# seung-lab/crackle

Hardware: AMD Instinct MI355X
Metric: voxels/s encode+decode, 1024x1024x512 uint32; bit-exact .ckl bytes (higher is better)
Workload: dtype u32

## Files before the change

### crackle_amd/_lib.py

```python
import ctypes as C
import os

HERE = os.path.dirname(os.path.abspath(__file__))
LIB_PATH = os.path.join(HERE, "libcrackle_amd_tuning.so" if os.environ.get("CKL_TUNING_LIB") else
                        ("libcrackle_amd_%s.so" % os.environ["CKL_LIB_AB"]) if os.environ.get("CKL_LIB_AB") else "libcrackle_amd.so")

CKL_OK, CKL_ERR_FORMAT, CKL_ERR_RUNTIME, CKL_ERR_ARG, CKL_ERR_NO_DEVICE, CKL_ERR_CRC = range(6)
MEM_HOST, MEM_DEVICE = 0, 1
CKL_DUST_BINARY_IMAGE, CKL_DUST_INVERT = 1, 2
CKL_ERODE_KEEP_BORDER = 1


class HeaderInfo(C.Structure):
  _fields_ = [
    ("format_version", C.c_uint32), ("label_format", C.c_uint32), ("crack_format", C.c_uint32),
    ("is_signed", C.c_uint32), ("data_width", C.c_uint32), ("stored_data_width", C.c_uint32),
    ("sx", C.c_uint32), ("sy", C.c_uint32), ("sz", C.c_uint32),
    ("fortran_order", C.c_uint32), ("markov_model_order", C.c_uint32), ("is_sorted", C.c_uint32),
    ("num_label_bytes", C.c_uint64), ("header_bytes", C.c_uint64),
  ]


MERGE_UNIQUE_FN = C.CFUNCTYPE(C.c_int, C.c_void_p, C.POINTER(C.c_uint64), C.c_uint64, C.POINTER(C.c_void_p), C.POINTER(C.c_uint64))

# ... 51 lines not shown
    C.c_int, C.c_int, C.c_uint64, C.c_int, C.c_int, C.c_int64,
    C.POINTER(EncodeOverrides), C.POINTER(C.c_void_p), C.POINTER(C.c_uint64)]),
  "ckl_encoder_stats": (C.c_int, [
    C.c_void_p, C.c_void_p, C.c_int64, C.c_int64, C.c_int64,
    C.POINTER(C.c_uint64), C.POINTER(C.c_uint64), C.POINTER(C.c_uint64), C.POINTER(C.c_uint64)]),
  "ckl_encoder_markov_stats": (C.c_int, [
    C.c_void_p, C.c_void_p, C.c_int64, C.c_int64, C.c_int64, C.c_int, C.c_uint64, C.c_void_p]),
  "ckl_encoder_components": (C.c_int, [
    C.c_void_p, C.c_void_p, C.c_int64, C.c_int64, C.c_int64, C.c_uint32, C.c_void_p, C.c_void_p]),
  "ckl_encoder_components_device": (C.c_int, [
    C.c_void_p, C.c_void_p, C.c_int64, C.c_int64, C.c_int64, C.c_uint32, C.c_void_p, C.c_void_p]),
  "ckl_encoder_pin_labels": (C.c_int, [
    C.c_void_p, C.c_void_p, C.c_void_p, C.c_int64, C.c_int64, C.c_int64, C.c_void_p,
    C.c_int, C.c_int, C.c_int64, C.POINTER(C.c_void_p), C.POINTER(C.c_uint64)]),
  "ckl_pins_rows_first": (C.c_int, [C.c_void_p, C.c_void_p, C.c_void_p, C.c_int64, C.c_int64, C.c_int64, C.c_int64, C.c_uint64, C.c_void_p, C.c_void_p, C.c_void_p]),
  "ckl_pins_rows_best": (C.c_int, [C.c_void_p, C.c_void_p, C.c_void_p, C.c_int64, C.c_int64, C.c_int64, C.c_int64, C.c_uint64, C.c_void_p, C.c_void_p]),
  "ckl_pins_rows_extent": (C.c_int, [C.c_void_p, C.c_void_p, C.c_void_p, C.c_int64, C.c_int64, C.c_int64, C.c_int64, C.c_uint64, C.c_void_p, C.c_void_p, C.c_void_p, C.c_void_p]),
  "ckl_pins_rows_ids": (C.c_int, [C.c_void_p, C.c_void_p, C.c_int64, C.c_int64, C.c_int64, C.c_int64, C.c_uint64, C.c_void_p, C.c_void_p, C.c_void_p, C.c_void_p]),
  "ckl_pins_rows_section": (C.c_int, [C.c_void_p, C.c_int64, C.c_int64, C.c_int64, C.c_uint64, C.c_void_p, C.c_void_p, C.c_void_p, C.c_void_p, C.c_void_p, C.c_void_p, C.c_void_p,
                                       C.c_int, C.c_int, C.c_int64, C.POINTER(C.c_void_p), C.POINTER(C.c_uint64)]),
  "ckl_encoder_walk_step_kinds": (C.c_int, [C.c_void_p, C.POINTER(C.c_uint32), C.c_uint32, C.POINTER(C.c_uint32)]),
  "ckl_encoder_last_timing": (C.c_int, [C.c_void_p, C.POINTER(C.c_float), C.POINTER(C.c_float)]),
  "ckl_encoder_walk_paths": (C.c_int, [C.c_void_p, C.POINTER(C.c_uint32), C.POINTER(C.c_uint32)]),
  "ckl_encoder_destroy": (None, [C.c_void_p]),
  "ckl_pin_labels_host": (C.c_int, [
    C.c_void_p, C.c_int, C.c_void_p, C.c_int64, C.c_int64, C.c_int64, C.c_void_p,
    C.c_int, C.c_int, C.c_int64, C.POINTER(C.c_void_p), C.POINTER(C.c_uint64)]),
  "ckl_zstack": (C.c_int, [C.POINTER(C.c_char_p), C.POINTER(C.c_uint64), C.c_uint64, C.POINTER(C.c_void_p), C.POINTER(C.c_uint64)]),
  "ckl_decoder_check": (C.c_int, [C.c_void_p, C.c_void_p, C.c_uint64]),
  "ckl_decoder_vcg": (C.c_int, [C.c_void_p, C.c_void_p, C.c_uint64, C.c_int]),
  "ckl_voxel_connectivity_graph": (C.c_int, [C.c_void_p, C.c_uint64, C.c_int, C.c_int, C.c_void_p, C.c_uint64]),
  "ckl_voxel_connectivity_graph_range": (C.c_int, [C.c_void_p, C.c_uint64, C.c_int64, C.c_int64, C.c_int, C.c_int, C.c_void_p, C.c_uint64]),
  "ckl_point_cloud": (C.c_int, [
    C.c_void_p, C.c_uint64, C.c_int64, C.c_int64, C.c_void_p, C.c_uint64, C.c_int, C.c_int, C.c_int,
    C.POINTER(C.c_void_p), C.POINTER(C.c_void_p), C.POINTER(C.c_void_p), C.POINTER(C.c_uint64)]),
  "ckl_reencode_markov": (C.c_int, [C.c_void_p, C.c_uint64, C.c_int, C.c_int, C.POINTER(C.c_void_p), C.POINTER(C.c_uint64)]),
  "ckl_recompress": (C.c_int, [C.c_void_p, C.c_uint64, C.c_int, C.c_int, C.POINTER(C.c_void_p), C.POINTER(C.c_uint64)]),
  "ckl_erode": (C.c_int, [C.c_void_p, C.c_uint64, C.c_int, C.c_int, C.c_int, C.c_int, C.POINTER(C.c_void_p), C.POINTER(C.c_uint64)]),
  "ckl_dilate": (C.c_int, [C.c_void_p, C.c_uint64, C.c_int, C.c_int, C.c_int, C.c_int, C.POINTER(C.c_void_p), C.POINTER(C.c_uint64)]),
  "ckl_decoder_crack_planes": (C.c_int, [C.c_void_p, C.POINTER(C.c_void_p), C.POINTER(C.c_void_p), C.POINTER(C.c_uint32), C.POINTER(C.c_uint64)]),
  "ckl_zsplit": (C.c_int, [C.c_void_p, C.c_uint64, C.c_int64, C.c_int64, C.POINTER(C.c_void_p), C.POINTER(C.c_uint64)]),
  "ckl_encoder_defer_codes": (C.c_int, [C.c_void_p, C.c_int]),
  "ckl_encoder_codes_to_host": (C.c_int, [C.c_void_p, C.c_void_p, C.c_uint64, C.POINTER(C.c_uint64)]),
  "ckl_host_register": (C.c_int, [C.c_void_p, C.c_uint64]),
  "ckl_host_unregister": (C.c_int, [C.c_void_p]),
  "ckl_array_equal": (C.c_int, [C.c_void_p, C.c_uint64, C.c_void_p, C.c_uint64, C.c_int, C.POINTER(C.c_int)]),
# ... 72 lines not shown
```

### crackle_amd/csrc/ckl_encode.hip

```cpp
#include "ckl_encoder.hpp"
#include "ckl_decoder.hpp"
#include "ckl_runs.hpp"
#include "ckl_strips.hpp"
#include "ckl_trail.hpp"
#include "ckl_recompress.hpp"

#include <algorithm>
#include <atomic>
#include <chrono>
#include <functional>
#include <memory>
#include <mutex>

namespace ckl {

using namespace dev;

template <typename LABEL>
__global__ void __launch_bounds__(kBlock) k_stats(const LABEL* __restrict__ labels, uint64_t voxels, unsigned long long* __restrict__ out ) {
	__shared__ unsigned long long s_max[kWaves], s_pairs[kWaves];
	unsigned long long mx = 0, pairs = 0;
	const uint64_t stride = static_cast<uint64_t>(gridDim.x) * kBlock;
	for (uint64_t i = static_cast<uint64_t>(blockIdx.x) * kBlock + threadIdx.x; i < voxels; i += stride) {
		const LABEL v = labels[i];
		if (static_cast<unsigned long long>(v) > mx) mx = v;
		if (i > 0) pairs += (labels[i - 1] == v);
	}
// ... 477 lines not shown
				const uint4 v = *reinterpret_cast<const uint4*>(fcode + g0);
				const uint32_t w4[4] = { v.x, v.y, v.z, v.w };
#pragma unroll
				for (uint32_t j = 0; j < 16; j++) c[j] = static_cast<uint8_t>(w4[j >> 2] >> (8u * (j & 3u)));
			}
			else {
#pragma unroll
				for (uint32_t j = 0; j < 16; j++) c[j] = g0 + j < nvalid ? fcode[g0 + j] : 0;
			}
			uint32_t prev = g0 ? fcode[g0 - 1] : 0u;
			uint32_t enc = 0;
#pragma unroll
			for (uint32_t j = 0; j < 16; j++) {
				if (g0 + j < nvalid) enc |= ((c[j] - prev) & 3u) << (2 * j);
				prev = c[j];
			}
			if (4u * w + 4u <= nbytes) reinterpret_cast<uint32_t*>(out)[w] = enc;
			else for (uint32_t k = 4u * w; k < nbytes; k++) out[k] = static_cast<uint8_t>(enc >> (8u * (k - 4u * w)));
		}
		if (tid == 0) a.payload_len[zi] = nbytes;
	}
}

__device__ __forceinline__ uint32_t markov_ctx(const uint8_t* d, uint32_t g, int order) {
	uint32_t ctx = 0;
	for (int j = 1; j <= order; j++) {
		const uint32_t v = (g >= static_cast<uint32_t>(j)) ? d[g - j] : 0u;
		ctx |= v << (2 * (order - j));
	}
	return ctx;
}

__global__ void __launch_bounds__(kBlock) k_markov_hist(
	const uint8_t* __restrict__ dcode, const uint64_t* __restrict__ cbase, const uint32_t* __restrict__ n_valid,
	int order, uint32_t* __restrict__ hist, uint32_t lds_entries
) {
	extern __shared__ uint32_t s_hist[];
	const uint32_t zi = blockIdx.x;
	const uint8_t* d = dcode + cbase[zi];
	const uint32_t n = n_valid[zi];
	const uint32_t entries = 4u << (2 * order);
	const bool local = entries <= lds_entries;
	if (local) {
		for (uint32_t i = threadIdx.x; i < entries; i += kBlock) s_hist[i] = 0;
		__syncthreads();
	}
// ... 665 lines not shown
	if (st && !po.empty()) *st = v;
	e.graph_permissible = on_device ? static_cast<int64_t>(v.pairs) < static_cast<int64_t>(static_cast<uint64_t>(sx) * sy * sz) / 2 : format == GraphFormat::PERMISSIBLE;
}

enum class CrackGoal { HISTOGRAM, CODES };
struct CrackRequest {
	CrackGoal goal = CrackGoal::CODES;
	bool permissible = false;
	int markov_order = 0;
	const std::vector<uint8_t>* model = nullptr;
	bool reuse_trail = false;
	std::function<void()> overlap;
};
struct CrackResult {
	std::vector<uint32_t> code_len;
	uint64_t total = 0;
	bool any_chain = false;
	std::vector<uint32_t> hist;
	std::vector<uint8_t> model;
};

inline size_t trail_walk_lds(uint32_t max_special) { return (static_cast<size_t>(max_special) + 256) * 16 + 1024; }

FinishArgs finish_args(const ckl_encoder& e, int64_t sx, int64_t sy, int markov_order) {
	FinishArgs fa;
	fa.sx = static_cast<int>(sx); fa.sy = static_cast<int>(sy);
	fa.xw = byte_width(static_cast<uint64_t>(sx) + 1); fa.yw = byte_width(static_cast<uint64_t>(sy) + 1);
	fa.markov = markov_order ? 1u : 0u;
	fa.cbase = e.d_cbase.p; fa.kbase = e.d_kbase.p;
	fa.n_chains = e.d_n_chains.p; fa.n_raw = e.d_n_raw.p; fa.n_valid = e.d_n_valid.p;
	fa.cp = e.d_cp.p; fa.chain_node = e.d_chain_node.p; fa.chain_off = e.d_chain_off.p; fa.chain_clen = e.d_chain_clen.p;
	fa.chain_order = e.d_chain_order.p; fa.chain_dst = e.d_chain_dst.p; fa.chain_vstart = e.d_chain_vstart.p;
	fa.fcode = e.d_fcode.p; fa.dcode = e.d_dcode.p;
	fa.pbase = e.d_pbase.p; fa.payload = e.d_payload.p; fa.bbase = e.d_bbase.p; fa.boc = e.d_boc.p;
	fa.payload_len = e.d_payload_len.p; fa.boc_len = e.d_boc_len.p;
	fa.z0 = 0;
	return fa;
}

TrailArgs trail_args(const ckl_encoder& e, int64_t sx, int64_t sy, uint32_t ns) {
	const uint64_t nverts = static_cast<uint64_t>(sx + 1) * (sy + 1);
	TrailArgs ta;
	ta.adjm = e.d_adjm.p; ta.adjm_stride = e.adjm_stride; ta.mtx2 = e.mtx2; ta.tiles_x = e.tiles_x; ta.tiles_y = e.tiles_y;
	ta.planeV = plane_v(e); ta.planeH = plane_h(e, ns); ta.row_words = e.row_words; ta.plane_words = e.plane_words;
	ta.sx = static_cast<uint32_t>(sx); ta.sy = static_cast<uint32_t>(sy); ta.inv = e.graph_permissible ? 0xFFFFFFFFu : 0u;
	ta.sxe = static_cast<uint32_t>(sx + 1); ta.sye = static_cast<uint32_t>(sy + 1); ta.nverts = static_cast<uint32_t>(nverts);
// ... 48 lines not shown
	const std::vector<uint32_t> errs = download(e.d_slice_err.p, ns, e.stream);
	for (uint32_t zi = 0; zi < ns; zi++) if (errs[zi]) throw Error(CKL_ERR_RUNTIME, "crackle_amd: crack walk scratch overflow on z=" + std::to_string(zi));
}

CrackResult crack_pass(ckl_encoder& e, int64_t sx, int64_t sy, int64_t sz, const CrackRequest& rq) {
	hipStream_t s = e.stream;
	const uint32_t ns = static_cast<uint32_t>(sz);
	const uint64_t nverts = static_cast<uint64_t>(sx + 1) * (sy + 1);
	const int markov_order = rq.markov_order;
	const bool reuse_trail = rq.reuse_trail;
	if (rq.goal == CrackGoal::HISTOGRAM && (!markov_order || rq.model)) throw Error(CKL_ERR_RUNTIME, "crackle_amd: internal: a markov histogram needs an order and no model");
	CrackResult result;
	e.d_slice_err.ensure(ns);
	const bool prezeroed = e.trail_zeroed && !reuse_trail;
	e.trail_zeroed = false;
	if (prezeroed) CKL_HIP(hipStreamWaitEvent(s, e.ev_prezero, 0));
	if (!reuse_trail && !prezeroed) CKL_HIP(hipMemsetAsync(e.d_slice_err.p, 0, ns * sizeof(uint32_t), s));

	std::vector<uint64_t> cbase(ns), sbase(ns), kbase(ns);
	std::vector<uint32_t> ccap(ns), scap(ns), kcap(ns), max_steps(ns);
	std::vector<uint64_t> nbase(ns), cobase(ns), ibase(ns);
	std::vector<uint32_t> ncap(ns), cocap(ns), icap(ns);
	uint64_t ctot = 0, stot = 0, ktot = 0, ntot = 0, cotot = 0, itot = 0;
	uint32_t max_ncap = 0, max_cocap = 0, max_icap = 0, max_special = 0;
	bool any = false;
	for (uint32_t zi = 0; zi < ns; zi++) {
		const uint64_t E = crack_edges(e, sx, sy, zi, rq.permissible);
		any = any || E > 0;
		const uint64_t cc = ((7 * E + 16 + 15) / 16) * 16;
		if (cc > 0xFFFFFFF0ull) throw Error(CKL_ERR_RUNTIME, "crackle_amd: slice has too many crack edges");
		cbase[zi] = ctot; ccap[zi] = static_cast<uint32_t>(cc); ctot += cc;
		max_steps[zi] = static_cast<uint32_t>(E + 1);
		const uint64_t nc = ((static_cast<uint64_t>(e.count_special[zi]) + e.count_corner[zi] + 16) / 16) * 16;
		if (nc >= (1ull << 28)) throw Error(CKL_ERR_RUNTIME, "crackle_amd: slice has too many crack vertices");
		nbase[zi] = ntot; ncap[zi] = static_cast<uint32_t>(nc); ntot += nc;
		cobase[zi] = cotot; cocap[zi] = e.count_corner[zi]; cotot += e.count_corner[zi];
		const uint64_t ic = 7 * nc + 16;
		ibase[zi] = itot; icap[zi] = static_cast<uint32_t>(ic); itot += ic;
		sbase[zi] = stot; scap[zi] = static_cast<uint32_t>(2 * nc + 4); stot += 2 * nc + 4;
		kbase[zi] = ktot; kcap[zi] = static_cast<uint32_t>(nc); ktot += nc;
		max_ncap = std::max<uint32_t>(max_ncap, ncap[zi]);
		max_cocap = std::max<uint32_t>(max_cocap, cocap[zi]);
		max_icap = std::max<uint32_t>(max_icap, icap[zi]);
		max_special = std::max<uint32_t>(max_special, e.count_special[zi]);
	}
	result.any_chain = any;
	if (g_ht && g_ht->on) {
		uint32_t over = 0;
		for (uint32_t zi = 0; zi < ns; zi++) over += e.count_special[zi] > 3584u;
		fprintf(stderr, "[ckl trail nodes] max special %u, slices above 3584: %u of %u\n", max_special, over, ns);
	}
	HT_MARK("c:caps");

	UploadPacker tables;
	tables.add(e.d_cbase, cbase); tables.add(e.d_ccap, ccap);
	tables.add(e.d_sbase, sbase); tables.add(e.d_scap, scap);
	tables.add(e.d_kbase, kbase); tables.add(e.d_kcap, kcap);
	e.d_cp.ensure(ctot); e.d_fcode.ensure(ctot);
	if (markov_order) e.d_dcode.ensure(ctot);
	e.d_stack_node.ensure(stot); e.d_stack_code.ensure(stot);
	e.d_chain_node.ensure(ktot); e.d_chain_off.ensure(ktot); e.d_chain_clen.ensure(ktot);
	e.d_chain_order.ensure(ktot); e.d_chain_dst.ensure(ktot); e.d_chain_vstart.ensure(ktot);
	e.d_n_chains.ensure(ns); e.d_n_raw.ensure(ns); e.d_n_valid.ensure(ns);
	e.d_payload_len.ensure(ns); e.d_boc_len.ensure(ns);
	const int xw = byte_width(static_cast<uint64_t>(sx) + 1), yw = byte_width(static_cast<uint64_t>(sy) + 1);
	std::vector<uint64_t> pbase(ns), bbase(ns);
	uint64_t ptot = 0, btot = 0;
	for (uint32_t zi = 0; zi < ns; zi++) {
		const uint64_t ncodes = ccap[zi];
		const uint64_t pbytes = markov_order ? (3ull * ncodes + 2 + 7) / 8 : (ncodes + 3) / 4;
		pbase[zi] = ptot; ptot += ((pbytes + 8 + 3) / 4) * 4;
		const uint64_t bbytes = 4 + yw + static_cast<uint64_t>(kcap[zi]) * (yw + 2 * xw);
		bbase[zi] = btot; btot += bbytes;
	}
	tables.add(e.d_pbase, pbase); tables.add(e.d_bbase, bbase);
	tables.add(e.t_nbase, nbase); tables.add(e.t_ncap, ncap);
	tables.add(e.t_cobase, cobase); tables.add(e.t_cocap, cocap);
	tables.add(e.t_ibase, ibase); tables.add(e.t_icap, icap);
	tables.add(e.t_max_steps, max_steps);
	tables.commit(e.d_crack_tables, s, e.uploads_by_kernel ? &e.tables_staging : nullptr);
	HT_MARK("c:tables");
	e.d_payload.ensure(ptot + 8); e.d_boc.ensure(btot + 8);
	e.codes_capacity = ptot + btot;
	if (markov_order) CKL_HIP(hipMemsetAsync(e.d_payload.p, 0, ptot + 8, s));

	DevBuf<unsigned long long> d_tdbg;
	size_t trail_lds_used = 0;
	if (!reuse_trail) {
		e.t_counters.ensure(7 * static_cast<size_t>(ns));
		if (!prezeroed) CKL_HIP(hipMemsetAsync(e.t_counters.p, 0, 7 * static_cast<size_t>(ns) * sizeof(uint32_t), s));
		e.t_node_vertex.ensure(ntot); e.t_node_adj.ensure(ntot + 16); e.t_vert2node.ensure(nverts * ns);
		e.t_corner_vertex.ensure(cotot);
		e.t_dart_end.ensure(4 * ntot); e.t_dart_len.ensure(4 * ntot); e.t_dart_minv.ensure(4 * ntot); e.t_dart_minpos.ensure(4 * ntot);
		e.t_dart_codes.ensure(4 * ntot); e.t_dart_inline.ensure(4 * ntot);
		e.t_parent.ensure(ntot); e.t_compmin.ensure(ntot); e.t_starts.ensure(ntot);
		const uint32_t start_words = static_cast<uint32_t>((nverts + 31) / 32);
		e.t_start_bits.ensure(static_cast<size_t>(start_words) * ns);
		if (!prezeroed) CKL_HIP(hipMemsetAsync(e.t_start_bits.p, 0, static_cast<size_t>(start_words) * ns * sizeof(uint32_t), s));
		e.t_items.ensure(itot); e.t_item_off.ensure(itot); e.t_chain_item0.ensure(ktot);
		e.t_events.ensure(itot); e.t_chain_ev0.ensure(ktot); e.t_ev_lnd.ensure(itot); e.t_ev_item.ensure(itot);
		e.last_trail_slices = ns;

		TrailArgs ta = trail_args(e, sx, sy, ns);
		const FinishArgs fa = finish_args(e, sx, sy, markov_order);
		if (kTuning && getenv("CKL_TRAIL_DIAG")) { d_tdbg.ensure(16); CKL_HIP(hipMemsetAsync(d_tdbg.p, 0, 128, s)); ta.dbg = d_tdbg.p; }
		int max_lds = 0;
		CKL_HIP(hipDeviceGetAttribute(&max_lds, hipDeviceAttributeMaxSharedMemoryPerBlock, e.device));
		const size_t budget = static_cast<size_t>(max_lds > 1024 ? max_lds - 1024 : 0);
		const uint32_t dart_blocks = (4 * max_ncap + kWalkChunk * kWaves - 1) / (kWalkChunk * kWaves);
		size_t clds = (static_cast<size_t>(max_special) + 1024) * 12;
		if (const char* env = getenv("CKL_TRAIL_LDS")) clds = static_cast<size_t>(std::max(0, atoi(env)));
		clds = (std::min(budget, std::max<size_t>(clds, 1024)) / 16) * 16;
		CKL_HIP(hipFuncSetAttribute(reinterpret_cast<const void*>(&k_trail_components), hipFuncAttributeMaxDynamicSharedMemorySize, static_cast<int>(clds)));
		size_t lds = trail_walk_lds(max_special);
		if (const char* env = getenv("CKL_TRAIL_LDS")) lds = static_cast<size_t>(std::max(0, atoi(env)));
		lds = std::min(budget, std::max<size_t>(lds, 4096));
		lds = (lds / 16) * 16;
		CKL_HIP(hipFuncSetAttribute(reinterpret_cast<const void*>(&k_trail_walk), hipFuncAttributeMaxDynamicSharedMemorySize, static_cast<int>(lds)));
		trail_lds_used = lds;
		HT_MARK("c:setup");

		if (any) {
			hipLaunchKernelGGL(k_trail_nodes, dim3(e.graph_blocks, ns), dim3(kBlock), 0, s, ta);
			hipLaunchKernelGGL(k_trail_segments, dim3(dart_blocks, ns), dim3(kBlock), 0, s, ta);
			if (max_cocap) hipLaunchKernelGGL(k_trail_loops, dim3((max_cocap + kBlock - 1) / kBlock, ns), dim3(kBlock), 0, s, ta);
			hipLaunchKernelGGL(k_trail_components, dim3(ns), dim3(kCompBlock), clds, s, ta, static_cast<uint32_t>(clds));
		}
		CKL_HIP(hipEventRecord(e.evd0, s));
		hipLaunchKernelGGL(k_trail_walk, dim3(ns), dim3(kWave), lds, s, ta, static_cast<uint32_t>(lds));
		CKL_HIP(hipEventRecord(e.evd1, s));
		hipLaunchKernelGGL(k_trail_items, dim3(ns), dim3(kItemsBlock), 0, s, ta);
		hipLaunchKernelGGL(k_trail_offsets, dim3(ns), dim3(kBlock), 0, s, ta);
		hipLaunchKernelGGL(k_trail_expand, dim3((max_icap + kExpandChunk * kWaves - 1) / (kExpandChunk * kWaves), ns), dim3(kBlock), 0, s, ta);
		hipLaunchKernelGGL(k_finish, dim3(ns), dim3(kFinishBlock), 0, s, fa);
	}
	HT_MARK("c:enqueue");
	if (kTuning && getenv("CKL_TRAIL_DIAG")) trail_diag(e, ns, d_tdbg.p, max_special, trail_lds_used);

	auto enqueue_tail = [&]() {
		e.d_out_off.ensure(ns);
		e.d_code_report.ensure(static_cast<size_t>(ns) + 3);
		e.d_codes_out.ensure(e.codes_capacity + 8);
		hipLaunchKernelGGL(k_code_offsets, dim3(1), dim3(kBlock), 0, s, e.d_boc_len.p, e.d_payload_len.p, e.d_slice_err.p, ns, e.d_out_off.p, e.d_code_report.p);
		hipLaunchKernelGGL(k_gather_codes, dim3(ns), dim3(kBlock), 0, s, e.d_boc.p, e.d_bbase.p, e.d_boc_len.p,
			e.d_payload.p, e.d_pbase.p, e.d_payload_len.p, e.d_out_off.p, e.d_codes_out.p);
	};
	if (!markov_order) enqueue_tail();
	if (rq.overlap) rq.overlap();
	HT_MARK("c:overlap");

	if (markov_order) {
		if (rq.model) result.model = *rq.model;
		else {
			const size_t rows = static_cast<size_t>(1) << (2 * markov_order);
			e.d_hist.ensure(rows * 4);
			CKL_HIP(hipMemsetAsync(e.d_hist.p, 0, rows * 4 * sizeof(uint32_t), s));
			const uint32_t hist_lds = (rows * 4 <= 16384) ? static_cast<uint32_t>(rows * 4) : 0u;
// ... 909 lines not shown
int ckl_encoder_last_timing(const ckl_encoder* e, float* pipeline_ms, float* dominant_kernel_ms) {
	if (!e) { set_last_error("crackle_amd: null encoder"); return CKL_ERR_ARG; }
	if (pipeline_ms) *pipeline_ms = e->pipeline_ms;
	if (dominant_kernel_ms) *dominant_kernel_ms = e->dominant_ms;
	return CKL_OK;
}

int ckl_encoder_walk_paths(ckl_encoder* e, uint32_t* fast_slices, uint32_t* compiled_slices) {
	return guard([&] {
		if (!e) throw Error(CKL_ERR_ARG, "crackle_amd: null encoder");
		uint32_t fast = 0, plain = 0;
		const size_t ns = e->last_trail_slices;
		if (ns && e->t_counters.p) {
			select_device(e->device);
			std::vector<uint32_t> nev(ns);
			CKL_HIP(hipMemcpy(nev.data(), e->t_counters.p + 5 * ns, ns * sizeof(uint32_t), hipMemcpyDeviceToHost));
			for (uint32_t v : nev) { if (v & (kEvFormatAddr12 | kEvWalkWide)) fast++; else if (v) plain++; }
		}
		if (fast_slices) *fast_slices = fast;
		if (compiled_slices) *compiled_slices = plain;
	});
}

int ckl_encoder_walk_step_kinds(ckl_encoder* e, uint32_t* counts, uint32_t max_slices, uint32_t* n_slices) {
	return guard([&] {
		if (!e || !counts || !n_slices) throw Error(CKL_ERR_ARG, "crackle_amd: null argument");
		const size_t ns = e->last_trail_slices;
		*n_slices = static_cast<uint32_t>(ns);
		if (!ns || !e->t_counters.p || !e->t_events.p) { *n_slices = 0; return; }
		if (ns > max_slices) throw Error(CKL_ERR_ARG, "crackle_amd: counts holds fewer slices than the last run had");
		select_device(e->device);
		DevBuf<uint32_t> d_counts;
		d_counts.ensure(ns * 5);
		hipLaunchKernelGGL(k_trail_step_kinds, dim3(static_cast<uint32_t>(ns)), dim3(kBlock), 0, e->stream, e->t_events.p, e->t_ibase.p, e->t_counters.p + 5 * ns, d_counts.p);
		CKL_HIP(hipMemcpyAsync(counts, d_counts.p, ns * 5 * sizeof(uint32_t), hipMemcpyDeviceToHost, e->stream));
		CKL_HIP(hipStreamSynchronize(e->stream));
	});
}

void ckl_encoder_destroy(ckl_encoder* e) { delete e; }

int ckl_compress(
	const void* labels, int labels_mem, int dtype_bytes, int is_signed,
	int64_t sx, int64_t sy, int64_t sz,
	int allow_pins, int fortran_order, uint64_t markov_model_order,
	int optimize_pins, int auto_bgcolor, int64_t manual_bgcolor,
// ... 32 lines not shown
```

### crackle_amd/csrc/ckl_encoder.hpp

```cpp
#pragma once

#include "ckl_common.hpp"

#include <chrono>
#include <utility>

struct VolumeStats { uint64_t max_label = 0, pairs = 0, first = 0, last = 0; };
namespace ckl { namespace dev { struct RunLabels; } }

struct ckl_encoder {
	template <typename T> using DevBuf = ckl::DevBuf<T>;

	int device = 0;
	hipStream_t stream = nullptr;
	hipStream_t stream2 = nullptr;
	hipEvent_t ev0 = nullptr, ev1 = nullptr, ev_in = nullptr;
	hipEvent_t evd0 = nullptr, evd1 = nullptr;
	hipEvent_t ev_prezero = nullptr;
	float pipeline_ms = 0.f, dominant_ms = 0.f;
	int dtype_bytes = 0;

	DevBuf<unsigned long long> d_stats;
	DevBuf<uint4> d_adjm;
	DevBuf<uint32_t> d_slice_err;
// ... 46 lines not shown
	std::vector<std::pair<const char*, double>> host_marks;
	VolumeStats planes_stats;
	int64_t planes_dims[3] = { 0, 0, 0 };
	std::vector<uint64_t> h_rbase;
	std::vector<uint32_t> h_rcap;
	std::vector<uint64_t> h_comp_off;
	DevBuf<uint16_t> s_run_lid, s_seam_first, s_seam_last;
	DevBuf<uint32_t> s_sc_w, s_sc_first, s_strip_nruns, s_strip_nsc;
	DevBuf<uint64_t> d_label_slots;
	uint32_t flat_nstrips = 0, flat_strip_rows = 0, flat_strip_cap = 0, flat_resolve_cap = 0;
	int max_lds = 0;
	bool flat_strips = false;
	std::vector<uint32_t> count_special, count_corner;
	DevBuf<uint32_t> d_plane_partial, t_blk_special, t_blk_corner;
	DevBuf<unsigned long long> d_plane_partial_max, d_plane_out;
	uint32_t graph_blocks = 0;
	uint32_t tiles_x = 0, tiles_y = 0, mtx2 = 0;
	uint64_t adjm_stride = 0;
	bool graph_permissible = false;
	bool planes_deferred = false;
	bool trail_zeroed = false;
	DevBuf<uint64_t> t_nbase, t_cobase, t_ibase;
	DevBuf<uint32_t> t_ncap, t_cocap, t_icap, t_max_steps;
	size_t last_trail_slices = 0;
	DevBuf<uint32_t> t_counters;
	DevBuf<uint32_t> t_node_vertex, t_vert2node, t_corner_vertex;
	DevBuf<uint8_t> t_node_adj;
	DevBuf<uint32_t> t_dart_end, t_dart_len, t_dart_minv, t_dart_minpos, t_parent, t_start_bits, t_starts;
	DevBuf<uint4> t_dart_codes;
	DevBuf<uint8_t> t_dart_inline;
	DevBuf<unsigned long long> t_compmin;
	DevBuf<uint32_t> t_items, t_item_off, t_chain_item0, t_events, t_chain_ev0, t_ev_lnd, t_ev_item;

	~ckl_encoder() {
		if (ev0) (void)hipEventDestroy(ev0);
		if (ev1) (void)hipEventDestroy(ev1);
		if (evd0) (void)hipEventDestroy(evd0);
		if (evd1) (void)hipEventDestroy(evd1);
		if (ev_in) (void)hipEventDestroy(ev_in);
		if (ev_prezero) (void)hipEventDestroy(ev_prezero);
		if (stream) (void)hipStreamDestroy(stream);
		if (stream2) (void)hipStreamDestroy(stream2);
		if (stream_copy) { (void)hipStreamSynchronize(stream_copy); (void)hipStreamDestroy(stream_copy); }
		if (stream_tab) { (void)hipStreamSynchronize(stream_tab); (void)hipStreamDestroy(stream_tab); }
		if (ev_codes) (void)hipEventDestroy(ev_codes);
		if (tables_staging) ckl::host_out_free(tables_staging);
// ... 85 lines not shown
```

### crackle_amd/distributed.py

```python
import ctypes as C
from typing import Optional, Sequence, Tuple

import numpy as np
import torch
import torch.distributed as dist

from . import _lib

FLAT = 0
IMPERMISSIBLE, PERMISSIBLE = 0, 1


def _byte_width(x: int) -> int:
  return 1 if x <= 0xFF else 2 if x <= 0xFFFF else 4 if x <= 0xFFFFFFFF else 8


def stats_to_model(hist: np.ndarray) -> np.ndarray:
  hist = np.asarray(hist, dtype=np.uint64).reshape(-1, 4)
  order = np.lexsort((-np.arange(4)[None, :].repeat(hist.shape[0], 0), -hist.astype(np.int64)), axis=1)
  model = np.empty_like(order, dtype=np.uint8)
  rows = np.arange(hist.shape[0])[:, None]
  model[rows, order] = np.arange(4, dtype=np.uint8)[None, :]
  return np.ascontiguousarray(model)

# ... 417 lines not shown
    return DeviceStream(p.value, n.value, owner=self, generation=self._stream_generation)

  def defer_codes(self, shape, itemsize: int, defer: bool):
    self._L.ckl_encoder_defer_codes(self._encoder(shape, itemsize), int(bool(defer)))

  def codes_to_host(self, dst_ptr: int, capacity: int) -> int:
    n = C.c_uint64()
    rc = self._L.ckl_encoder_codes_to_host(self._enc, dst_ptr, capacity, C.byref(n))
    if rc != _lib.CKL_OK:
      raise RuntimeError(_lib.last_error())
    return int(n.value)

  def encoder_timing(self) -> Tuple[float, float]:
    p, k = C.c_float(), C.c_float()
    if self._enc:
      self._L.ckl_encoder_last_timing(self._enc, C.byref(p), C.byref(k))
    return p.value, k.value

  def walk_paths(self) -> Tuple[int, int]:
    f, c = C.c_uint32(), C.c_uint32()
    if self._enc and self._L.ckl_encoder_walk_paths(self._enc, C.byref(f), C.byref(c)) != _lib.CKL_OK:
      raise RuntimeError(_lib.last_error())
    return f.value, c.value

  def walk_step_kinds(self, max_slices: int = 1 << 16):
    buf = (C.c_uint32 * (5 * max_slices))()
    n = C.c_uint32()
    if not self._enc:
      return np.zeros((0, 5), np.uint32)
    if self._L.ckl_encoder_walk_step_kinds(self._enc, buf, max_slices, C.byref(n)) != _lib.CKL_OK:
      raise RuntimeError(_lib.last_error())
    return np.frombuffer(buf, dtype=np.uint32, count=5 * n.value).reshape(n.value, 5).copy()

  def open_decoder(self, binary: bytes, z_start: int, z_end: int):
    return HipDecodeSession(binary, z_start, z_end, self.device_index)

  def __del__(self):
    try:
      if self._enc:
        self._L.ckl_encoder_destroy(self._enc)
    except Exception:
      pass


class ShardedCodec:

# ... 488 lines not shown
```

### include/crackle_amd.h

```cpp
#ifndef CRACKLE_AMD_H
#define CRACKLE_AMD_H

#include <stdint.h>

#ifdef __cplusplus
extern "C" {
#endif

typedef enum ckl_status {
	CKL_OK = 0,
	CKL_ERR_FORMAT = 1,
	CKL_ERR_RUNTIME = 2,
	CKL_ERR_ARG = 3,
	CKL_ERR_NO_DEVICE = 4,
	CKL_ERR_CRC = 5
} ckl_status;

enum { CKL_MEM_HOST = 0, CKL_MEM_DEVICE = 1 };

const char* ckl_last_error(void);

int ckl_abi_version(void);

int ckl_device_count(void);
// ... 130 lines not shown
	ckl_encoder* e, const void* labels_device, int64_t sx, int64_t sy, int64_t sz,
	uint32_t id_base, uint32_t* cc_device, uint32_t* ncomp_host);

int ckl_encoder_pin_labels(
	ckl_encoder* e, const void* labels_device, const uint32_t* cc_device,
	int64_t sx, int64_t sy, int64_t sz, const uint32_t* ncomp_host,
	int stored_width, int auto_bgcolor, int64_t manual_bgcolor,
	uint8_t** out, uint64_t* out_len);

int ckl_pins_rows_first(ckl_encoder* e, const void* labels_rows, const uint32_t* cc_rows, int64_t sx, int64_t rows, int64_t sz, int64_t y0,
	uint64_t n_components, uint64_t* first_any, uint64_t* first_kept, uint64_t* comp_label);
int ckl_pins_rows_best(ckl_encoder* e, const void* labels_rows, const uint32_t* cc_rows, int64_t sx, int64_t rows, int64_t sz, int64_t y0,
	uint64_t n_components, const uint64_t* first_kept, uint64_t* best);
int ckl_pins_rows_extent(ckl_encoder* e, const void* labels_rows, const uint32_t* cc_rows, int64_t sx, int64_t rows, int64_t sz, int64_t y0,
	uint64_t n_components, const uint64_t* first_kept, const uint64_t* best, uint64_t* choice, uint32_t* ze_plus1);
int ckl_pins_rows_ids(ckl_encoder* e, const uint32_t* cc_rows, int64_t sx, int64_t rows, int64_t sz, int64_t y0,
	uint64_t n_components, const uint64_t* choice, const uint32_t* ze_plus1, const uint64_t* offsets, uint32_t* ids);
int ckl_pins_rows_section(ckl_encoder* e, int64_t sx, int64_t sy, int64_t sz, uint64_t n_components, const uint32_t* ncomp_host,
	const uint64_t* comp_label, const uint64_t* first_any, const uint64_t* choice, const uint32_t* ze_plus1, const uint64_t* offsets, const uint32_t* ids,
	int stored_width, int auto_bgcolor, int64_t manual_bgcolor, uint8_t** out, uint64_t* out_len);

int ckl_encoder_last_timing(const ckl_encoder* e, float* pipeline_ms, float* dominant_kernel_ms);
int ckl_encoder_walk_paths(ckl_encoder* e, uint32_t* fast_slices, uint32_t* compiled_slices);
int ckl_encoder_walk_step_kinds(ckl_encoder* e, uint32_t* counts, uint32_t max_slices, uint32_t* n_slices);
void ckl_encoder_destroy(ckl_encoder* e);


int ckl_zstack(
	const uint8_t* const* bufs, const uint64_t* lens, uint64_t count,
	uint8_t** out, uint64_t* out_len);

int ckl_pin_labels_host(
	const void* labels, int dtype_bytes, const uint32_t* cc,
	int64_t sx, int64_t sy, int64_t sz, const uint32_t* ncomp,
	int stored_width, int auto_bgcolor, int64_t manual_bgcolor,
	uint8_t** out, uint64_t* out_len);

int ckl_point_cloud(
	const uint8_t* buf, uint64_t n, int64_t z_start, int64_t z_end,
	const uint64_t* labels, uint64_t n_labels, int has_labels, int skip_background, int device,
	uint64_t** labels_out, uint64_t** offsets_out, uint16_t** points_out, uint64_t* n_out);

int ckl_reencode_markov(const uint8_t* buf, uint64_t n, int markov_model_order, int device, uint8_t** out, uint64_t* out_len);

int ckl_recompress(const uint8_t* buf, uint64_t n, int markov_model_order, int device, uint8_t** out, uint64_t* out_len);

// ... 34 lines not shown
```

Measured before the change: 160.0 billion.

## Fuse trail offsets, expand and finish into one LDS-resident emit kernel

Replaces the three-kernel sequence (k_trail_offsets, k_trail_expand, k_finish) with a single per-slice k_trail_emit kernel. It computes item offsets with a block scan, writes the chain index, and places 2-bit crack codes directly into packed words in LDS. Inline dart codes are OR-ed in as shifted 128-bit chunks, and long darts are walked by dedicated waves. The packed diff is then computed with SWAR arithmetic instead of a per-code difference pass. This removes the intermediate cp/fcode global buffers and two kernel launches. The cost is one 1024-thread block per slice, a serial single-thread chain sort and index build, heavy LDS use, and atomics on shared words.

```diff
diff --git a/crackle_amd/_lib.py b/crackle_amd/_lib.py
--- a/crackle_amd/_lib.py
+++ b/crackle_amd/_lib.py
@@ -97,6 +97,7 @@
   "ckl_encoder_walk_step_kinds": (C.c_int, [C.c_void_p, C.POINTER(C.c_uint32), C.c_uint32, C.POINTER(C.c_uint32)]),
   "ckl_encoder_last_timing": (C.c_int, [C.c_void_p, C.POINTER(C.c_float), C.POINTER(C.c_float)]),
   "ckl_encoder_walk_paths": (C.c_int, [C.c_void_p, C.POINTER(C.c_uint32), C.POINTER(C.c_uint32)]),
+  "ckl_encoder_emit_path": (C.c_int, [C.c_void_p, C.POINTER(C.c_int), C.POINTER(C.c_uint64)]),
   "ckl_encoder_destroy": (None, [C.c_void_p]),
   "ckl_pin_labels_host": (C.c_int, [
     C.c_void_p, C.c_int, C.c_void_p, C.c_int64, C.c_int64, C.c_int64, C.c_void_p,
diff --git a/crackle_amd/csrc/ckl_code_words.hpp b/crackle_amd/csrc/ckl_code_words.hpp
--- /dev/null
+++ b/crackle_amd/csrc/ckl_code_words.hpp
@@ -0,0 +1,37 @@
+#pragma once
+
+#include <cstdint>
+
+#if defined(__HIPCC__)
+#define CKL_HOST_DEVICE __host__ __device__
+#else
+#define CKL_HOST_DEVICE
+#endif
+
+namespace ckl {
+
+CKL_HOST_DEVICE inline uint32_t place_codes128(const uint32_t (&q)[4], uint32_t len, uint32_t index, uint32_t (&out)[5]) {
+	uint32_t m[4];
+	for (uint32_t j = 0; j < 4; j++) {
+		const uint32_t bits = 2u * len > 32u * j ? 2u * len - 32u * j : 0u;
+		m[j] = q[j] & (bits >= 32u ? 0xFFFFFFFFu : (1u << bits) - 1u);
+	}
+	const uint32_t s = 2u * (index & 15u);
+	if (s == 0u) { out[0] = m[0]; out[1] = m[1]; out[2] = m[2]; out[3] = m[3]; out[4] = 0u; }
+	else {
+		out[0] = m[0] << s;
+		out[1] = (m[1] << s) | (m[0] >> (32u - s));
+		out[2] = (m[2] << s) | (m[1] >> (32u - s));
+		out[3] = (m[3] << s) | (m[2] >> (32u - s));
+		out[4] = m[3] >> (32u - s);
+	}
+	return index >> 4;
+}
+
+CKL_HOST_DEVICE inline uint32_t packed_code_diff(uint32_t word, uint32_t prev_top) {
+	constexpr uint32_t H = 0xAAAAAAAAu;
+	const uint32_t pred = (word << 2) | (prev_top & 3u);
+	return ((word | H) - (pred & ~H)) ^ ((word ^ ~pred) & H);
+}
+
+}
diff --git a/crackle_amd/csrc/ckl_encode.hip b/crackle_amd/csrc/ckl_encode.hip
--- a/crackle_amd/csrc/ckl_encode.hip
+++ b/crackle_amd/csrc/ckl_encode.hip
@@ -3,6 +3,7 @@
 #include "ckl_runs.hpp"
 #include "ckl_strips.hpp"
 #include "ckl_trail.hpp"
+#include "ckl_code_words.hpp"
 #include "ckl_recompress.hpp"
 
 #include <algorithm>
@@ -526,6 +527,250 @@
 	}
 }
 
+constexpr int kEmitBlock = 1024;
+constexpr int kEmitWaves = kEmitBlock / kWave;
+constexpr uint32_t kEmitLong = 1024;
+
+struct EmitSlice {
+	uint32_t zi, n, nch, total, wcap;
+	const uint32_t* items;
+	const uint32_t* off;
+	const uint32_t* dlen;
+	uint64_t nb;
+};
+
+__device__ __forceinline__ void emit_chains_and_codes(
+	const TrailArgs& a, const FinishArgs& f, const EmitSlice& sl, uint32_t* words,
+	const uint32_t* ch_node, const uint32_t* item0, const uint32_t* vstart, uint32_t* order, uint32_t* dst,
+	const uint32_t* s_long, const uint32_t* s_nlong, uint32_t* s_carry
+) {
+	const uint32_t tid = threadIdx.x;
+	const uint32_t zi = sl.zi, n = sl.n, nch = sl.nch, total = sl.total;
+	const uint32_t sxe = f.sx + 1;
+
+	if (tid == 0) {
+		auto clen = [&](uint32_t c) -> uint32_t { return (c + 1 < nch ? vstart[c + 1] : total) - vstart[c]; };
+		for (uint32_t c = 0; c < nch; c++) {
+			const uint32_t key = ch_node[c];
+			uint32_t p = c;
+			while (p > 0 && ch_node[order[p - 1]] > key) { order[p] = order[p - 1]; p--; }
+			order[p] = c;
+		}
+		uint32_t d = 0;
+		for (uint32_t i = 0; i < nch; i++) { dst[order[i]] = d; d += clen(order[i]); }
+
+		uint8_t* b = f.boc + f.bbase[zi];
+		uint32_t num_y = 0, index_size = f.yw;
+		for (uint32_t i = 0; i < nch;) {
+			const uint32_t y = ch_node[order[i]] / sxe;
+			uint32_t j = i;
+			while (j < nch && ch_node[order[j]] / sxe == y) j++;
+			index_size += f.yw + (j - i + 1) * f.xw;
+			num_y++;
+			i = j;
+		}
+		uint32_t idx = 0;
+		put_le_dev(b + idx, index_size, 4); idx += 4;
+		put_le_dev(b + idx, num_y, f.yw); idx += f.yw;
+		uint32_t last_y = 0;
+		for (uint32_t i = 0; i < nch;) {
+			const uint32_t y = ch_node[order[i]] / sxe;
+			uint32_t j = i;
+			while (j < nch && ch_node[order[j]] / sxe == y) j++;
+			put_le_dev(b + idx, y - last_y, f.yw); idx += f.yw;
+			last_y = y;
+			put_le_dev(b + idx, j - i, f.xw); idx += f.xw;
+			uint32_t last_x = 0;
+			for (uint32_t k = i; k < j; k++) {
+				const uint32_t x = ch_node[order[k]] - sxe * y;
+				put_le_dev(b + idx, x - last_x, f.xw); idx += f.xw;
+				last_x = x;
+			}
+			i = j;
+		}
+		f.boc_len[zi] = idx;
+		a.n_raw[zi] = total; a.n_valid[zi] = total;
+		*s_carry = 0;
+	}
+	__syncthreads();
+	__threadfence_block();
+	for (uint32_t c = tid; c < nch; c += kEmitBlock) dst[c] -= vstart[c];
+	__syncthreads();
+	__threadfence_block();
+
+	const uint32_t nwords = (total + 15u) >> 4, nbytes = (total + 3u) >> 2;
+	const uint4* adjm = a.adjm + zi * a.adjm_stride;
+	uint8_t* out = f.payload + f.pbase[zi];
+	uint8_t* dcode = f.dcode + a.cbase[zi];
+	const uint32_t nl = *s_nlong;
+	const bool listed = nl <= kEmitLong;
+	const uint32_t walkers = listed ? min((nl + kWave - 1u) / kWave, static_cast<uint32_t>(kEmitWaves / 2)) * kWave : 0u;
+	for (uint32_t w0 = 0; w0 < nwords; w0 += sl.wcap) {
+		const uint32_t wn = min(sl.wcap, nwords - w0);
+		for (uint32_t i = tid; i < wn; i += kEmitBlock) words[i] = 0u;
+		__syncthreads();
+		auto or_word = [&](uint32_t gw, uint32_t v) {
+			const uint32_t wi = gw - w0;
+			if (v && wi < wn) atomicOr(words + wi, v);
+		};
+		auto place = [&](uint32_t i) -> uint32_t {
+			uint32_t lo = 0, hi = nch;
+			while (hi - lo > 1u) { const uint32_t mid = (lo + hi) >> 1; if (item0[mid] <= i) lo = mid; else hi = mid; }
+			return sl.off[i] + dst[lo];
+		};
+		auto outside = [&](uint32_t p, uint32_t len) -> bool { return (p >> 4) >= w0 + wn || ((p + len - 1u) >> 4) < w0; };
+		auto walk = [&](uint32_t d, uint32_t p, uint32_t len) {
+			const uint32_t v0 = a.node_vertex[sl.nb + (d >> 2)];
+			uint32_t y = v0 / a.sxe, x = v0 - y * a.sxe, k = d & 3u, acc = 0u;
+			MicroTile c;
+			c.lo = c.hi = make_uint4(0, 0, 0, 0); c.mx = c.my = 0xFFFFFFFFu;
+			for (uint32_t s = 0; s < len; s++) {
+				const uint32_t g = p + s;
+				acc |= trail_code(k) << (2u * (g & 15u));
+				if ((g & 15u) == 15u || s + 1u == len) { or_word(g >> 4, acc); acc = 0u; }
+				trail_step(x, y, k);
+				if (s + 1u == len) break;
+				if (x > a.sx || y > a.sy) { atomicOr(a.slice_err + zi, TRAIL_ERR_CAPACITY); break; }
+				if (!c.holds(x, y)) mt_load(c, adjm, x, y, a.mtx2);
+				k = (__ffs(c.nib(x, y) & ~(1u << (k ^ 1u))) - 1) & 3u;
+			}
+		};
+		if (tid < walkers) {
+			for (uint32_t j = tid; j < nl; j += walkers) {
+				const uint32_t i = s_long[j];
+				const uint32_t d = sl.items[i] & ~kItemMask, len = sl.dlen[d], p = place(i);
+				if (!outside(p, len)) walk(d, p, len);
+			}
+		}
+		else {
+			for (uint32_t i = tid - walkers; i < n; i += kEmitBlock - walkers) {
+				const uint32_t it = sl.items[i], kind = it & kItemMask;
+				if (kind != kItemSeg && kind != kItemCtl) continue;
+				const uint32_t p = place(i);
+				if (kind == kItemCtl) { or_word(p >> 4, (it & 3u) << (2u * (p & 15u))); or_word((p + 1u) >> 4, ((it >> 2) & 3u) << (2u * ((p + 1u) & 15u))); continue; }
+				const uint32_t d = it & ~kItemMask;
+				const uint32_t len = sl.dlen[d];
+				if (len == 0u || outside(p, len)) continue;
+				if (len <= kInlineCodes && a.dart_inline[sl.nb * 4u + d]) {
+					const uint4 q4 = a.dart_codes[sl.nb * 4u + d];
+					const uint32_t q[4] = { q4.x, q4.y, q4.z, q4.w };
+					uint32_t o[5];
+					const uint32_t gw = place_codes128(q, len, p, o);
+#pragma unroll
+					for (uint32_t j = 0; j < 5; j++) or_word(gw + j, o[j]);
+				}
+				else if (!listed) walk(d, p, len);
+			}
+		}
+		__syncthreads();
+		for (uint32_t i = tid; i < wn; i += kEmitBlock) {
+			const uint32_t gw = w0 + i;
+			uint32_t enc = packed_code_diff(words[i], i ? words[i - 1] >> 30 : *s_carry);
+			if (gw == nwords - 1u && (total & 15u)) enc &= (1u << (2u * (total & 15u))) - 1u;
+			if (f.markov) {
+				auto spread = [](uint32_t b) -> uint32_t { uint32_t x = (b | (b << 12)) & 0x000F000Fu; return (x | (x << 6)) & 0x03030303u; };
+				*reinterpret_cast<uint4*>(dcode + 16ull * gw) = make_uint4(spread(enc & 255u), spread((enc >> 8) & 255u), spread((enc >> 16) & 255u), spread(enc >> 24));
+			}
+			else if (4u * gw + 4u <= nbytes) reinterpret_cast<uint32_t*>(out)[gw] = enc;
+			else for (uint32_t k = 4u * gw; k < nbytes; k++) out[k] = static_cast<uint8_t>(enc >> (8u * (k - 4u * gw)));
+		}
+		__syncthreads();
+		if (tid == 0) *s_carry = words[wn - 1u] >> 30;
+		__syncthreads();
+	}
+	if (tid == 0) f.payload_len[zi] = f.markov ? 0u : nbytes;
+}
+
+__global__ void __launch_bounds__(kEmitBlock, 8) k_trail_emit(TrailArgs a, FinishArgs f, uint32_t tcap, uint32_t wcap) {
+	extern __shared__ uint32_t s_emit[];
+	__shared__ uint32_t s_scan[kEmitWaves];
+	__shared__ uint32_t s_long[kEmitLong];
+	__shared__ uint32_t s_nlong, s_carry;
+	const uint32_t zi = blockIdx.x + a.z0;
+	const uint32_t tid = threadIdx.x;
+	if (a.slice_err[zi]) {
+		if (tid == 0) { a.n_raw[zi] = 0; a.n_valid[zi] = 0; f.payload_len[zi] = 0; f.boc_len[zi] = 0; }
+		return;
+	}
+	const uint32_t n = a.n_items[zi];
+	const uint32_t nch = a.n_chains[zi];
+	const uint64_t nb = a.nbase[zi], kb = a.kbase[zi];
+	const uint32_t* items = a.items + a.ibase[zi];
+	uint32_t* off = a.item_off + a.ibase[zi];
+	const uint32_t* dlen = a.dart_len + nb * 4u;
+	const uint8_t* dinl = a.dart_inline + nb * 4u;
+	if (tid == 0) s_nlong = 0u;
+	__syncthreads();
+
+	uint32_t total = 0;
+	{
+		constexpr uint32_t kPer = 4;
+		for (uint32_t i0 = 0; i0 < n; i0 += kEmitBlock * kPer) {
+			uint32_t len[kPer], cnt = 0;
+#pragma unroll
+			for (uint32_t q = 0; q < kPer; q++) {
+				const uint32_t i = i0 + tid * kPer + q;
+				len[q] = 0;
+				if (i < n) {
+					const uint32_t it = items[i];
+					const uint32_t kind = it & kItemMask;
+					if (kind == kItemSeg) {
+						const uint32_t d = it & ~kItemMask;
+						len[q] = dlen[d];
+						if (len[q] > kInlineCodes || (len[q] && !dinl[d])) {
+							const uint32_t j = atomicAdd(&s_nlong, 1u);
+							if (j < kEmitLong) s_long[j] = i;
+						}
+					}
+					else if (kind == kItemCtl) len[q] = 2u;
+				}
+				cnt += len[q];
+			}
+			uint32_t v[1] = { cnt }, tot[1];
+			block_excl_add<1, kEmitWaves>(v, tot, s_scan);
+			uint32_t o = total + v[0];
+#pragma unroll
+			for (uint32_t q = 0; q < kPer; q++) {
+				const uint32_t i = i0 + tid * kPer + q;
+				if (i < n) off[i] = o;
+				o += len[q];
+			}
+			total += tot[0];
+		}
+	}
+	__syncthreads();
+	__threadfence_block();
+	if (total > a.ccap[zi]) {
+		if (tid == 0) { atomicOr(a.slice_err + zi, TRAIL_ERR_CAPACITY); a.n_raw[zi] = total; a.n_valid[zi] = total; f.payload_len[zi] = 0; f.boc_len[zi] = 0; }
+		return;
+	}
+
+	const EmitSlice sl = { zi, n, nch, total, wcap, items, off, dlen, nb };
+	uint32_t* words = s_emit + 2u * tcap;
+	const uint32_t* g_node = a.chain_node + kb;
+	const uint32_t* g_item0 = a.chain_item0 + kb;
+	if (nch <= tcap) {
+		uint32_t* s_item0 = s_emit;
+		uint32_t* s_dst = s_emit + tcap;
+		uint32_t* s_node = words;
+		uint32_t* s_order = words + tcap;
+		uint32_t* s_vstart = words + 2u * tcap;
+		for (uint32_t c = tid; c < nch; c += kEmitBlock) {
+			const uint32_t i0 = g_item0[c];
+			s_item0[c] = i0; s_node[c] = g_node[c]; s_vstart[c] = i0 < n ? off[i0] : total;
+		}
+		__syncthreads();
+		emit_chains_and_codes(a, f, sl, words, s_node, s_item0, s_vstart, s_order, s_dst, s_long, &s_nlong, &s_carry);
+	}
+	else {
+		uint32_t* g_vstart = a.chain_off + kb;
+		for (uint32_t c = tid; c < nch; c += kEmitBlock) { const uint32_t i0 = g_item0[c]; g_vstart[c] = i0 < n ? off[i0] : total; }
+		__syncthreads();
+		__threadfence_block();
+		emit_chains_and_codes(a, f, sl, words, g_node, g_item0, g_vstart, f.chain_order + kb, f.chain_dst + kb, s_long, &s_nlong, &s_carry);
+	}
+}
+
 __device__ __forceinline__ uint32_t markov_ctx(const uint8_t* d, uint32_t g, int order) {
 	uint32_t ctx = 0;
 	for (int j = 1; j <= order; j++) {
@@ -1237,6 +1482,33 @@
 
 inline size_t trail_walk_lds(uint32_t max_special) { return (static_cast<size_t>(max_special) + 256) * 16 + 1024; }
 
+constexpr size_t kEmitLdsCap = 80 * 1024;
+struct EmitPlan {
+	bool fused = false;
+	uint32_t tcap = 0, wcap = 0;
+	size_t dyn = 0, need = 0;
+};
+EmitPlan emit_plan(uint64_t max_edges, uint32_t max_kcap, int max_lds) {
+	EmitPlan p;
+	static const size_t static_lds = [] {
+		hipFuncAttributes fattr;
+		CKL_HIP(hipFuncGetAttributes(&fattr, reinterpret_cast<const void*>(&k_trail_emit)));
+		return static_cast<size_t>(fattr.sharedSizeBytes);
+	}();
+	p.tcap = std::min<uint32_t>(kFinishChains, ((max_kcap + 15u) / 16u) * 16u);
+	const uint64_t words = (max_edges + max_edges / 8 + 1024 + 15) / 16;
+	p.wcap = static_cast<uint32_t>(std::min<uint64_t>(words, 1u << 28));
+	if (const char* env = getenv("CKL_TRAIL_EMIT_WORDS")) p.wcap = static_cast<uint32_t>(std::max(1, std::min<int>(atoi(env), static_cast<int>(p.wcap))));
+	p.dyn = 4 * (2 * static_cast<size_t>(p.tcap) + std::max<size_t>(3 * static_cast<size_t>(p.tcap), p.wcap));
+	p.need = static_lds + p.dyn;
+	size_t cap = kEmitLdsCap;
+	if (const char* env = getenv("CKL_TRAIL_EMIT_LDS")) cap = static_cast<size_t>(std::max(0, atoi(env)));
+	cap = std::min(cap, static_cast<size_t>(std::max(0, max_lds)));
+	const char* sw = getenv("CKL_TRAIL_EMIT");
+	p.fused = !(sw && !strcmp(sw, "0")) && words < (1u << 28) && p.need <= cap;
+	return p;
+}
+
 FinishArgs finish_args(const ckl_encoder& e, int64_t sx, int64_t sy, int markov_order) {
 	FinishArgs fa;
 	fa.sx = static_cast<int>(sx); fa.sy = static_cast<int>(sy);
@@ -1331,7 +1603,8 @@
 	std::vector<uint64_t> nbase(ns), cobase(ns), ibase(ns);
 	std::vector<uint32_t> ncap(ns), cocap(ns), icap(ns);
 	uint64_t ctot = 0, stot = 0, ktot = 0, ntot = 0, cotot = 0, itot = 0;
-	uint32_t max_ncap = 0, max_cocap = 0, max_icap = 0, max_special = 0;
+	uint32_t max_ncap = 0, max_cocap = 0, max_icap = 0, max_special = 0, max_kcap = 0;
+	uint64_t max_edges = 0;
 	bool any = false;
 	for (uint32_t zi = 0; zi < ns; zi++) {
 		const uint64_t E = crack_edges(e, sx, sy, zi, rq.permissible);
@@ -1352,6 +1625,8 @@
 		max_cocap = std::max<uint32_t>(max_cocap, cocap[zi]);
 		max_icap = std::max<uint32_t>(max_icap, icap[zi]);
 		max_special = std::max<uint32_t>(max_special, e.count_special[zi]);
+		max_kcap = std::max<uint32_t>(max_kcap, kcap[zi]);
+		max_edges = std::max<uint64_t>(max_edges, E);
 	}
 	result.any_chain = any;
 	if (g_ht && g_ht->on) {
@@ -1365,11 +1640,18 @@
 	tables.add(e.d_cbase, cbase); tables.add(e.d_ccap, ccap);
 	tables.add(e.d_sbase, sbase); tables.add(e.d_scap, scap);
 	tables.add(e.d_kbase, kbase); tables.add(e.d_kcap, kcap);
-	e.d_cp.ensure(ctot); e.d_fcode.ensure(ctot);
+	int max_lds = 0;
+	CKL_HIP(hipDeviceGetAttribute(&max_lds, hipDeviceAttributeMaxSharedMemoryPerBlock, e.device));
+	EmitPlan emit;
+	if (!reuse_trail) {
+		emit = emit_plan(max_edges, max_kcap, max_lds);
+		e.emit_fused = emit.fused; e.emit_lds = emit.need;
+		if (!emit.fused) { e.d_cp.ensure(ctot); e.d_fcode.ensure(ctot); e.d_chain_clen.ensure(ktot); e.d_chain_vstart.ensure(ktot); }
+	}
 	if (markov_order) e.d_dcode.ensure(ctot);
 	e.d_stack_node.ensure(stot); e.d_stack_code.ensure(stot);
-	e.d_chain_node.ensure(ktot); e.d_chain_off.ensure(ktot); e.d_chain_clen.ensure(ktot);
-	e.d_chain_order.ensure(ktot); e.d_chain_dst.ensure(ktot); e.d_chain_vstart.ensure(ktot);
+	e.d_chain_node.ensure(ktot); e.d_chain_off.ensure(ktot);
+	e.d_chain_order.ensure(ktot); e.d_chain_dst.ensure(ktot);
 	e.d_n_chains.ensure(ns); e.d_n_raw.ensure(ns); e.d_n_valid.ensure(ns);
 	e.d_payload_len.ensure(ns); e.d_boc_len.ensure(ns);
 	const int xw = byte_width(static_cast<uint64_t>(sx) + 1), yw = byte_width(static_cast<uint64_t>(sy) + 1);
@@ -1413,8 +1695,6 @@
 		TrailArgs ta = trail_args(e, sx, sy, ns);
 		const FinishArgs fa = finish_args(e, sx, sy, markov_order);
 		if (kTuning && getenv("CKL_TRAIL_DIAG")) { d_tdbg.ensure(16); CKL_HIP(hipMemsetAsync(d_tdbg.p, 0, 128, s)); ta.dbg = d_tdbg.p; }
-		int max_lds = 0;
-		CKL_HIP(hipDeviceGetAttribute(&max_lds, hipDeviceAttributeMaxSharedMemoryPerBlock, e.device));
 		const size_t budget = static_cast<size_t>(max_lds > 1024 ? max_lds - 1024 : 0);
 		const uint32_t dart_blocks = (4 * max_ncap + kWalkChunk * kWaves - 1) / (kWalkChunk * kWaves);
 		size_t clds = (static_cast<size_t>(max_special) + 1024) * 12;
@@ -1439,9 +1719,15 @@
 		hipLaunchKernelGGL(k_trail_walk, dim3(ns), dim3(kWave), lds, s, ta, static_cast<uint32_t>(lds));
 		CKL_HIP(hipEventRecord(e.evd1, s));
 		hipLaunchKernelGGL(k_trail_items, dim3(ns), dim3(kItemsBlock), 0, s, ta);
-		hipLaunchKernelGGL(k_trail_offsets, dim3(ns), dim3(kBlock), 0, s, ta);
-		hipLaunchKernelGGL(k_trail_expand, dim3((max_icap + kExpandChunk * kWaves - 1) / (kExpandChunk * kWaves), ns), dim3(kBlock), 0, s, ta);
-		hipLaunchKernelGGL(k_finish, dim3(ns), dim3(kFinishBlock), 0, s, fa);
+		if (emit.fused) {
+			CKL_HIP(hipFuncSetAttribute(reinterpret_cast<const void*>(&k_trail_emit), hipFuncAttributeMaxDynamicSharedMemorySize, static_cast<int>(emit.dyn)));
+			hipLaunchKernelGGL(k_trail_emit, dim3(ns), dim3(kEmitBlock), emit.dyn, s, ta, fa, emit.tcap, emit.wcap);
+		}
+		else {
+			hipLaunchKernelGGL(k_trail_offsets, dim3(ns), dim3(kBlock), 0, s, ta);
+			hipLaunchKernelGGL(k_trail_expand, dim3((max_icap + kExpandChunk * kWaves - 1) / (kExpandChunk * kWaves), ns), dim3(kBlock), 0, s, ta);
+			hipLaunchKernelGGL(k_finish, dim3(ns), dim3(kFinishBlock), 0, s, fa);
+		}
 	}
 	HT_MARK("c:enqueue");
 	if (kTuning && getenv("CKL_TRAIL_DIAG")) trail_diag(e, ns, d_tdbg.p, max_special, trail_lds_used);
@@ -2397,6 +2683,13 @@
 	});
 }
 
+int ckl_encoder_emit_path(const ckl_encoder* e, int* fused, uint64_t* lds_bytes) {
+	if (!e) { set_last_error("crackle_amd: null encoder"); return CKL_ERR_ARG; }
+	if (fused) *fused = e->emit_fused ? 1 : 0;
+	if (lds_bytes) *lds_bytes = e->emit_lds;
+	return CKL_OK;
+}
+
 int ckl_encoder_walk_step_kinds(ckl_encoder* e, uint32_t* counts, uint32_t max_slices, uint32_t* n_slices) {
 	return guard([&] {
 		if (!e || !counts || !n_slices) throw Error(CKL_ERR_ARG, "crackle_amd: null argument");
diff --git a/crackle_amd/csrc/ckl_encoder.hpp b/crackle_amd/csrc/ckl_encoder.hpp
--- a/crackle_amd/csrc/ckl_encoder.hpp
+++ b/crackle_amd/csrc/ckl_encoder.hpp
@@ -92,6 +92,8 @@
 	bool trail_zeroed = false;
 	DevBuf<uint64_t> t_nbase, t_cobase, t_ibase;
 	DevBuf<uint32_t> t_ncap, t_cocap, t_icap, t_max_steps;
+	bool emit_fused = false;
+	size_t emit_lds = 0;
 	size_t last_trail_slices = 0;
 	DevBuf<uint32_t> t_counters;
 	DevBuf<uint32_t> t_node_vertex, t_vert2node, t_corner_vertex;
diff --git a/crackle_amd/distributed.py b/crackle_amd/distributed.py
--- a/crackle_amd/distributed.py
+++ b/crackle_amd/distributed.py
@@ -463,6 +463,12 @@
     if self._enc and self._L.ckl_encoder_walk_paths(self._enc, C.byref(f), C.byref(c)) != _lib.CKL_OK:
       raise RuntimeError(_lib.last_error())
     return f.value, c.value
+
+  def emit_path(self) -> Tuple[bool, int]:
+    f, n = C.c_int(), C.c_uint64()
+    if self._enc and self._L.ckl_encoder_emit_path(self._enc, C.byref(f), C.byref(n)) != _lib.CKL_OK:
+      raise RuntimeError(_lib.last_error())
+    return bool(f.value), int(n.value)
 
   def walk_step_kinds(self, max_slices: int = 1 << 16):
     buf = (C.c_uint32 * (5 * max_slices))()
diff --git a/include/crackle_amd.h b/include/crackle_amd.h
--- a/include/crackle_amd.h
+++ b/include/crackle_amd.h
@@ -176,6 +176,7 @@
 
 int ckl_encoder_last_timing(const ckl_encoder* e, float* pipeline_ms, float* dominant_kernel_ms);
 int ckl_encoder_walk_paths(ckl_encoder* e, uint32_t* fast_slices, uint32_t* compiled_slices);
+int ckl_encoder_emit_path(const ckl_encoder* e, int* fused, uint64_t* lds_bytes);
 int ckl_encoder_walk_step_kinds(ckl_encoder* e, uint32_t* counts, uint32_t max_slices, uint32_t* n_slices);
 void ckl_encoder_destroy(ckl_encoder* e);
 
```

New measurement: 167.5 billion, median of 6. 4.7% higher.
